# silencht/SG-SLAM

Hardware: AMD Instinct MI355X
Metric: tracked frames/sec (640x480 RGB-D) (higher is better)
Workload: dtype u8/f32(bf16x3 matrix products)/f64

## Files before the change

sg_slam_amd/csrc/sgx_flow.cpp:

```cpp
#include "sgx_flow_kernels.h"
#include "sgx_prof.h"
#include "sgx_stage.h"
#include "../../include/sgx.h"
#ifdef SGX_DEBUG_TAPS
#include "../../include/sgx_debug.h"
#endif
#include <stdio.h>
#include <stdlib.h>
#include <string.h>
#include <new>
#include <vector>

#define SGX_CHECK_HIP(expr) do { hipError_t _e = (expr); if (_e != hipSuccess) { \
    fprintf(stderr, "sgx: HIP error %d (%s) at %s:%d\n", (int)_e, hipGetErrorString(_e), __FILE__, __LINE__); return SGX_ERR_DEVICE; } } while (0)

struct sgx_flow {
    sgx_flow_config cfg;
    SgxLkGeom g;
    uint8_t *img[2] = { nullptr, nullptr };
    int cur = 0;
    int prev_batch = 0;
};

extern "C" int sgx_flow_create(const sgx_flow_config *cfg, sgx_flow **out)
{
    if (!cfg || !out) return SGX_ERR_INVALID;
    *out = nullptr;
    if (cfg->width < 1 || cfg->height < 1 || cfg->max_batch < 1 || cfg->max_count < 0 || !(cfg->epsilon >= 0)) return SGX_ERR_INVALID;
    if (cfg->win_size != SGX_LK_WIN || cfg->max_level < 0 || cfg->max_level >= SGX_LK_MAXL) return SGX_ERR_UNSUPPORTED;
    if (cfg->width <= 1 || cfg->height <= 1) return SGX_ERR_UNSUPPORTED;
    { const unsigned long long qw = (unsigned long long)((cfg->width + 3) >> 2); if (qw * qw * (unsigned long long)cfg->height >= (1ull << 32)) return SGX_ERR_UNSUPPORTED; }
    sgx_flow *h = new (std::nothrow) sgx_flow();
    if (!h) return SGX_ERR_NOMEM;
    h->cfg = *cfg;
    SgxLkGeom &g = h->g;
    memset(&g, 0, sizeof g);
    int w = cfg->width, hh = cfg->height; unsigned io = 0;
    for (int l = 0;; l++) {
        g.w[l] = w; g.h[l] = hh; g.pitch[l] = (w + 3) & ~3; g.ioff[l] = io;
        io += (unsigned)g.pitch[l] * (unsigned)hh;
        g.nl = l + 1;
        if (l == cfg->max_level) break;
        const int nw = (w + 1) / 2, nh = (hh + 1) / 2;
        if (nw <= cfg->win_size || nh <= cfg->win_size) break;
        w = nw; hh = nh;
    }
    g.img_stride = (io + 15u + 64u) & ~15u;
    for (int s = 0; s < 2; s++)
        if (hipMalloc((void **)&h->img[s], (size_t)g.img_stride * cfg->max_batch) != hipSuccess) { sgx_flow_destroy(h); return SGX_ERR_NOMEM; }
    *out = h;
    return SGX_OK;
}

extern "C" void sgx_flow_destroy(sgx_flow *h)
{
    if (!h) return;
    for (int s = 0; s < 2; s++) if (h->img[s]) (void)hipFree(h->img[s]);
    delete h;
}

extern "C" int sgx_flow_reset(sgx_flow *h) { if (!h) return SGX_ERR_INVALID; h->prev_batch = 0; return SGX_OK; }
extern "C" int sgx_flow_levels(const sgx_flow *h) { return h ? h->g.nl : SGX_ERR_INVALID; }

static int build_pyramid(sgx_flow *h, int slot, const uint8_t *d_gray, int pitch, int batch, sgx_stream_t st)
{
    const SgxLkGeom &g = h->g;
    uint8_t *base = h->img[slot];
    sgx_prof_begin(SGX_K_LK_PYR, st);
    auto magic = [](int d) -> unsigned { return d <= 1 ? 0u : (unsigned)((0x100000000ull + (unsigned)d - 1) / (unsigned)d); };
    SGX_LAUNCH(k_lk_copy, dim3(((g.pitch[0] >> 2) * g.h[0] + 255) / 256, batch), dim3(256), st, d_gray, g.w[0], g.h[0], pitch, base, g.pitch[0], g.img_stride, magic(g.pitch[0] >> 2));
    for (int l = 1; l < g.nl; l++)
        SGX_LAUNCH(k_lk_pyrdown, dim3(((g.pitch[l] >> 2) * g.h[l] + 255) / 256, batch), dim3(256), st, (const uint8_t *)(base + g.ioff[l - 1]), g.w[l - 1], g.h[l - 1], g.pitch[l - 1],
                   g.img_stride, base + g.ioff[l], g.w[l], g.h[l], g.pitch[l], g.img_stride, magic(g.pitch[l] >> 2));
    sgx_prof_end(SGX_K_LK_PYR, st);
    SGX_CHECK_HIP(hipGetLastError());
    return SGX_OK;
}

static int track(sgx_flow *h, int cur_slot, int prev_slot, int batch, const sgx_keypoint *d_keys, const int32_t *d_n, int cap, float *d_prev_xy, uint8_t *d_status, sgx_stream_t st)
{
    SgxLkArgs A;
    A.cur_img = h->img[cur_slot]; A.prev_img = h->img[prev_slot];
    A.keys = (const uint8_t *)d_keys; A.n = d_n; A.cap = cap; A.prev_xy = d_prev_xy; A.status = d_status;
    A.max_count = h->cfg.max_count > 100 ? 100 : h->cfg.max_count;
    double eps = h->cfg.epsilon > 10. ? 10. : h->cfg.epsilon;
    A.eps2 = eps * eps; A.min_eig = (float)1e-4;
    sgx_prof_begin(SGX_K_LK_TRACK, st);
    static const int kpw = sgx_getenv("SGX_LK_KPW") ? atoi(sgx_getenv("SGX_LK_KPW")) : 2;
    A.batch = batch; A.kblocks = (cap + 4 * kpw - 1) / (4 * kpw);
#ifdef SGX_DEBUG_TAPS
    if (kpw == 4) { auto kfn = k_lk_trackN<4>; SGX_LAUNCH(kfn, dim3((unsigned)A.kblocks * (unsigned)batch), dim3(256), st, h->g, A); }
    else if (kpw != 2) { A.kblocks = (cap + 3) / 4; SGX_LAUNCH(k_lk_track, dim3((unsigned)A.kblocks * (unsigned)batch), dim3(256), st, h->g, A); }
    else
#endif
    { auto kfn = k_lk_trackN<2>; SGX_LAUNCH(kfn, dim3((unsigned)A.kblocks * (unsigned)batch), dim3(256), st, h->g, A); }
    sgx_prof_end(SGX_K_LK_TRACK, st);
    SGX_CHECK_HIP(hipGetLastError());
    return SGX_OK;
}

extern "C" int sgx_flow_lk_batch_dev(sgx_flow *h, const uint8_t *d_gray, int pitch, int batch, const sgx_keypoint *d_keys, const int32_t *d_n, int cap,
                                     float *d_prev_xy, uint8_t *d_status, int32_t *have_prev, void *stream)
{
    if (!h || !d_gray || batch < 1 || batch > h->cfg.max_batch || pitch < h->cfg.width) return SGX_ERR_INVALID;
    if ((pitch & 3) || ((uintptr_t)d_gray & 3)) return SGX_ERR_INVALID;
    sgx_stream_t st = (sgx_stream_t)stream;
    const int cur = h->cur, prev = cur ^ 1;
    const bool tracked = h->prev_batch == batch;
    if (tracked && (!d_keys || !d_n || !d_prev_xy || cap < 1)) return SGX_ERR_INVALID;
    int rc = build_pyramid(h, cur, d_gray, pitch, batch, st);
    if (rc != SGX_OK) return rc;
    if (tracked) { rc = track(h, cur, prev, batch, d_keys, d_n, cap, d_prev_xy, d_status, st); if (rc != SGX_OK) return rc; }
    if (have_prev) *have_prev = tracked ? 1 : 0;
    h->cur = prev; h->prev_batch = batch;
    return SGX_OK;
}

extern "C" int sgx_flow_lk(sgx_flow *h, const uint8_t *gray_from, const uint8_t *gray_to, int stride, const float *pts, int n, float *next_pts, uint8_t *status)
{
    if (!h || !gray_from || !gray_to || stride < h->cfg.width || n < 0 || (n > 0 && (!pts || !next_pts))) return SGX_ERR_INVALID;
    if (n == 0) return SGX_OK;
    const int W = h->cfg.width, H = h->cfg.height, P = (W + 3) & ~3;
    std::vector<uint8_t> pack((size_t)P * H * 2, 0);
    for (int y = 0; y < H; y++) { memcpy(&pack[(size_t)y * P], gray_to + (size_t)y * stride, (size_t)W); memcpy(&pack[(size_t)(H + y) * P], gray_from + (size_t)y * stride, (size_t)W); }
    std::vector<sgx_keypoint> kp((size_t)n);
    for (int i = 0; i < n; i++) { memset(&kp[(size_t)i], 0, sizeof(sgx_keypoint)); kp[(size_t)i].x = pts[2 * i]; kp[(size_t)i].y = pts[2 * i + 1]; }
    SgxStaged dI, dK, dN, dO, dS;
    int rc;
    if ((rc = dI.put(0, pack.data(), pack.size())) != SGX_OK || (rc = dK.put(1, kp.data(), kp.size() * sizeof(sgx_keypoint))) != SGX_OK ||
        (rc = dN.put(2, &n, sizeof n)) != SGX_OK || (rc = dO.put(3, nullptr, (size_t)n * 8)) != SGX_OK || (rc = dS.put(4, nullptr, (size_t)n)) != SGX_OK) return rc;
    const int keep_cur = h->cur, keep_prev = h->prev_batch;
    if ((rc = build_pyramid(h, 1, (const uint8_t *)dI.p, P, 1, 0)) != SGX_OK) return rc;
    if ((rc = build_pyramid(h, 0, (const uint8_t *)dI.p + (size_t)P * H, P, 1, 0)) != SGX_OK) return rc;
    if ((rc = track(h, 0, 1, 1, (const sgx_keypoint *)dK.p, (const int32_t *)dN.p, n, (float *)dO.p, (uint8_t *)dS.p, 0)) != SGX_OK) return rc;
    SGX_CHECK_HIP(hipMemcpy(next_pts, dO.p, (size_t)n * 8, hipMemcpyDeviceToHost));
    if (status) SGX_CHECK_HIP(hipMemcpy(status, dS.p, (size_t)n, hipMemcpyDeviceToHost));
    h->cur = keep_cur; h->prev_batch = 0; (void)keep_prev;
    return SGX_OK;
}

SGX_TAP int sgx_flow_debug_read_level(sgx_flow *h, int slot, int frame, int level, uint8_t *img )
{
    if (!h || slot < 0 || slot > 1 || frame < 0 || frame >= h->cfg.max_batch || level < 0 || level >= h->g.nl) return SGX_ERR_INVALID;
    const SgxLkGeom &g = h->g;
    SGX_CHECK_HIP(hipDeviceSynchronize());
    if (!img) return SGX_ERR_INVALID;
    {
        std::vector<uint8_t> t((size_t)g.pitch[level] * g.h[level]);
        SGX_CHECK_HIP(hipMemcpy(t.data(), h->img[slot] + (size_t)frame * g.img_stride + g.ioff[level], t.size(), hipMemcpyDeviceToHost));
        for (int y = 0; y < g.h[level]; y++) memcpy(img + (size_t)y * g.w[level], &t[(size_t)y * g.pitch[level]], (size_t)g.w[level]);
    }
    return SGX_OK;
}
SGX_TAP int sgx_flow_debug_level_size(const sgx_flow *h, int level, int32_t *w, int32_t *hh)
{
    if (!h || level < 0 || level >= h->g.nl || !w || !hh) return SGX_ERR_INVALID;
    *w = h->g.w[level]; *hh = h->g.h[level];
    return SGX_OK;
}

#if defined(SGX_DEBUG_TAPS) && !defined(SGX_EMU)
typedef float sgx_dbg_f16v __attribute__((ext_vector_type(16)));
typedef __bf16 sgx_dbg_bf8 __attribute__((ext_vector_type(8)));
SGX_KERNEL_OCC(256, 2) k_dbg_corun_bf16(float *o, int iters)
{
    const uint32_t x = threadIdx.x * 2654435761u + blockIdx.x, y = x ^ 0x9e3779b9u;
    sgx_dbg_f16v acc = {0}; sgx_dbg_bf8 a, b;
    for (int i = 0; i < 8; i++) { a[i] = (__bf16)(float)((x >> i) & 7); b[i] = (__bf16)(float)((y >> i) & 3); }
    for (int i = 0; i < iters; i++) acc = __builtin_amdgcn_mfma_f32_32x32x16_bf16(a, b, acc, 0, 0, 0);
    float s = 0.f; for (int i = 0; i < 16; i++) s += acc[i];
    o[(blockIdx.x & 1023) * 256 + threadIdx.x] = s;
}
#endif
SGX_TAP int sgx_debug_corun_bf16(int blocks, int iters, int launches, void *stream)
{
#if defined(SGX_DEBUG_TAPS) && !defined(SGX_EMU)
    static float *sink = nullptr;
    if (blocks < 1 || iters < 1 || launches < 1) return SGX_ERR_INVALID;
    if (!sink) SGX_CHECK_HIP(hipMalloc((void **)&sink, 1024 * 256 * sizeof(float)));
    for (int l = 0; l < launches; l++) SGX_LAUNCH(k_dbg_corun_bf16, dim3((unsigned)blocks), dim3(256), (sgx_stream_t)stream, sink, iters);
    SGX_CHECK_HIP(hipGetLastError());
    return SGX_OK;
#else
    (void)blocks; (void)iters; (void)launches; (void)stream;
    return SGX_ERR_UNSUPPORTED;
#endif
}

extern "C" int sgx_fundamental_ransac_batch_dev(int batch, int cap, const sgx_keypoint *d_keys, const int32_t *d_n, const float *d_prev_xy,
                                                const int32_t *d_pre_have_dynamic, const float *d_pre_boxes, const int32_t *d_pre_nboxes, int max_boxes,
                                                double threshold, double confidence, double *d_F, int32_t *d_ok, int32_t *d_stats, void *stream)
{
    if (batch < 1 || cap < 1 || !d_keys || !d_n || !d_prev_xy || !d_F || !d_ok || max_boxes < 0) return SGX_ERR_INVALID;
    if (cap > SGX_FM_MAXPTS) return SGX_ERR_UNSUPPORTED;
    SgxFmArgs A;
    A.keys = (const uint8_t *)d_keys; A.n = d_n; A.cap = cap; A.prev_xy = d_prev_xy;
    A.pre_have = d_pre_have_dynamic; A.pre_boxes = d_pre_boxes; A.pre_nboxes = d_pre_nboxes; A.max_boxes = max_boxes;
    if (threshold <= 0) threshold = 3;
    if (confidence < DBL_EPSILON || confidence > 1 - DBL_EPSILON) confidence = 0.99;
    A.threshold = threshold; A.confidence = confidence; A.max_iters = 1000;
    A.F = d_F; A.ok = d_ok; A.stats = d_stats;
    const size_t lds = (size_t)cap * 16 + 1024 + (((size_t)cap + 15) & ~(size_t)15);
    sgx_prof_begin(SGX_K_FM_RANSAC, (sgx_stream_t)stream);
    SGX_LAUNCH_DYN(k_fm_ransac, dim3(batch), dim3(256), lds, (sgx_stream_t)stream, A);
    sgx_prof_end(SGX_K_FM_RANSAC, (sgx_stream_t)stream);
    SGX_CHECK_HIP(hipGetLastError());
    return SGX_OK;
}

extern "C" int sgx_find_fundamental_mat(const float *pts1, const float *pts2, int n, double threshold, double confidence, double *F, int32_t *ok, int32_t *stats)
{
    if (n < 0 || (n > 0 && (!pts1 || !pts2)) || !F || !ok) return SGX_ERR_INVALID;
    if (n > SGX_FM_MAXPTS) return SGX_ERR_UNSUPPORTED;
    const int cap = n > 0 ? n : 1;
    std::vector<sgx_keypoint> kp((size_t)cap);
    memset(kp.data(), 0, kp.size() * sizeof(sgx_keypoint));
    for (int i = 0; i < n; i++) { kp[(size_t)i].x = pts1[2 * i]; kp[(size_t)i].y = pts1[2 * i + 1]; }
    SgxStaged dK, dN, dP, dF, dO, dS;
    int rc;
    if ((rc = dK.put(0, kp.data(), kp.size() * sizeof(sgx_keypoint))) != SGX_OK || (rc = dN.put(1, &n, sizeof n)) != SGX_OK ||
        (rc = dP.put(2, n ? pts2 : nullptr, (size_t)cap * 8)) != SGX_OK || (rc = dF.put(3, nullptr, 72)) != SGX_OK || (rc = dO.put(4, nullptr, 4)) != SGX_OK ||
        (rc = dS.put(5, nullptr, 16)) != SGX_OK) return rc;
    rc = sgx_fundamental_ransac_batch_dev(1, cap, (const sgx_keypoint *)dK.p, (const int32_t *)dN.p, (const float *)dP.p, nullptr, nullptr, nullptr, 0, threshold, confidence,
                                          (double *)dF.p, (int32_t *)dO.p, (int32_t *)dS.p, nullptr);
    if (rc != SGX_OK) return rc;
    SGX_CHECK_HIP(hipMemcpy(F, dF.p, 72, hipMemcpyDeviceToHost));
    SGX_CHECK_HIP(hipMemcpy(ok, dO.p, 4, hipMemcpyDeviceToHost));
    if (stats) SGX_CHECK_HIP(hipMemcpy(stats, dS.p, 16, hipMemcpyDeviceToHost));
    return SGX_OK;
}
```

sg_slam_amd/csrc/sgx_flow_kernels.h:

```cpp
#pragma once
#include "sgx_rt.h"
#include "sgx_block.h"
#include <float.h>
#include <math.h>

#define SGX_LK_MAXL 4
#define SGX_LK_WIN 21
#define SGX_LK_TILE_PITCH 36
struct SgxLkGeom {
    int nl;
    int w[SGX_LK_MAXL], h[SGX_LK_MAXL], pitch[SGX_LK_MAXL];
    unsigned ioff[SGX_LK_MAXL];
    unsigned img_stride;
};

SGX_DEV int sgx_reflect101(int p, int len)
{
    if (len == 1) return 0;
    while (p < 0 || p >= len) { if (p < 0) p = -p; else p = 2 * len - 2 - p; }
    return p;
}
SGX_DEV int sgx_floor_f(float v) { return (int)floorf(v); }
SGX_DEV float sgx_i64_to_f32(long long v)
{
    const long long hi = v >> 24; const int lo = (int)(v - (hi << 24));
    return (float)(int)hi * 16777216.0f + (float)lo;
}

SGX_DEV unsigned sgx_lk_udiv(unsigned n, unsigned m)
{
#ifndef SGX_EMU
    return m ? __umulhi(n, m) : n;
#else
    return m ? (unsigned)(((unsigned long long)n * m) >> 32) : n;
#endif
}
SGX_KERNEL(256) k_lk_copy(const uint8_t *src, int w, int h, int spitch, uint8_t *dst, int dpitch, unsigned dstride, unsigned qw_magic)
{
    SGX_THREADS_BEGIN(tid)
    const int f = (int)blockIdx.y, qw = dpitch >> 2, q = (int)blockIdx.x * 256 + tid;
    if (q < qw * h) {
        const int y = (int)sgx_lk_udiv((unsigned)q, qw_magic), x = (q - y * qw) * 4;
        const uint8_t *s = src + ((size_t)f * h + y) * spitch;
        uint32_t v;
        if (x + 4 <= w) v = *(const uint32_t *)(s + x);
        else { v = 0; for (int i = 0; x + i < w; i++) v |= (uint32_t)s[x + i] << (8 * i); }
        *(uint32_t *)(dst + (size_t)f * dstride + (size_t)y * dpitch + x) = v;
    }
    SGX_THREADS_END
}

SGX_KERNEL(256) k_lk_pyrdown(const uint8_t *src, int sw, int sh, int spitch, unsigned sstride, uint8_t *dst, int dw, int dh, int dpitch, unsigned dstride, unsigned qw_magic)
{
    SGX_THREADS_BEGIN(tid)
    const int f = (int)blockIdx.y, qw = dpitch >> 2, q = (int)blockIdx.x * 256 + tid;
    if (q < qw * dh) {
        const int y = (int)sgx_lk_udiv((unsigned)q, qw_magic), X = (q - y * qw) * 4;
        const uint8_t *S = src + (size_t)f * sstride;
        int acc[4] = { 0, 0, 0, 0 };
        const bool fast = X >= 2 && 2 * X + 11 < spitch && 2 * X + 8 <= sw - 1;
#pragma unroll
        for (int k = 0; k < 5; k++) {
            const int wk = k == 0 || k == 4 ? 1 : k == 2 ? 6 : 4;
            const uint8_t *row = S + (size_t)sgx_reflect101(2 * y - 2 + k, sh) * spitch;
            int p[11];
            if (fast) {
                const uint32_t *r4 = (const uint32_t *)(row + 2 * X - 4);
                const uint32_t a = r4[0], b = r4[1], c = r4[2], d = r4[3];
                p[0] = (a >> 16) & 255; p[1] = a >> 24;
                p[2] = b & 255; p[3] = (b >> 8) & 255; p[4] = (b >> 16) & 255; p[5] = b >> 24;
                p[6] = c & 255; p[7] = (c >> 8) & 255; p[8] = (c >> 16) & 255; p[9] = c >> 24;
                p[10] = d & 255;
            } else {
#pragma unroll
                for (int i = 0; i < 11; i++) p[i] = row[sgx_reflect101(2 * X - 2 + i, sw)];
            }
#pragma unroll
            for (int o = 0; o < 4; o++) acc[o] += wk * (p[2 * o + 2] * 6 + (p[2 * o + 1] + p[2 * o + 3]) * 4 + p[2 * o] + p[2 * o + 4]);
        }
        uint32_t out = 0;
#pragma unroll
        for (int o = 0; o < 4; o++) out |= (uint32_t)((acc[o] + 128) >> 8) << (8 * o);
        *(uint32_t *)(dst + (size_t)f * dstride + (size_t)y * dpitch + X) = out;
    }
    SGX_THREADS_END
}

struct SgxLkWeights { int w00, w01, w10, w11; };
SGX_DEV SgxLkWeights sgx_lk_weights(float a, float b)
{
    SgxLkWeights k;
    k.w00 = sgx_cvround((1.f - a) * (1.f - b) * (float)(1 << 14));
    k.w01 = sgx_cvround(a * (1.f - b) * (float)(1 << 14));
    k.w10 = sgx_cvround((1.f - a) * b * (float)(1 << 14));
    k.w11 = (1 << 14) - k.w00 - k.w01 - k.w10;
    return k;
}
#define SGX_LK_DESCALE(x, n) (((x) + (1 << ((n) - 1))) >> (n))

struct SgxLkStep { float dx, dy; };
SGX_DEV SgxLkStep sgx_lk_step(float A11, float A12, float A22, float D, long long sb1, long long sb2)
{
    const float FLT_SCALE = 1.f / (1 << 20);
    const float b1 = sgx_i64_to_f32(sb1) * FLT_SCALE, b2 = sgx_i64_to_f32(sb2) * FLT_SCALE;
    SgxLkStep s;
    s.dx = (A12 * b2 - A22 * b1) * D;
    s.dy = (A12 * b1 - A11 * b2) * D;
    return s;
}

struct SgxLkArgs {
    const uint8_t *cur_img, *prev_img;
    const uint8_t *keys; const int *n; int cap;
    float *prev_xy; uint8_t *status;
    int max_count; double eps2; float min_eig;
    int batch, kblocks;
};
SGX_DEV void sgx_lk_decode_block(int i, int batch, int kblocks, int &f, int &kb)
{
    const int full = (batch / 8) * 8;
    if (i < full * kblocks) { const int x = i & 7, j = i >> 3; kb = j % kblocks; f = x + 8 * (j / kblocks); }
    else { const int j = i - full * kblocks; f = full + j / kblocks; kb = j % kblocks; }
}

#ifdef SGX_EMU
static inline int sgx_lk_px(const uint8_t *I, int w, int h, int pitch, int x, int y) { return I[(size_t)sgx_reflect101(y, h) * pitch + sgx_reflect101(x, w)]; }
static void sgx_lk_track_point(const SgxLkGeom &g, const uint8_t *I0, const uint8_t *J0, float kx, float ky, int max_count, double eps2, float min_eig,
                               float *ox, float *oy, uint8_t *ost)
{
    const int W = SGX_LK_WIN; const float half = (W - 1) * 0.5f, FLT_SCALE = 1.f / (1 << 20);
    float outx = 0.f, outy = 0.f; uint8_t status = 1;
    static thread_local short Iw[SGX_LK_WIN * SGX_LK_WIN], dIw[SGX_LK_WIN * SGX_LK_WIN * 2];
    for (int level = g.nl - 1; level >= 0; level--) {
        const int w = g.w[level], h = g.h[level], pitch = g.pitch[level];
        const uint8_t *I = I0 + g.ioff[level], *J = J0 + g.ioff[level];
        const float sc = 1.0f / (float)(1 << level);
        float prevx = kx * sc, prevy = ky * sc, nextx, nexty;
        if (level == g.nl - 1) { nextx = prevx; nexty = prevy; } else { nextx = outx * 2.f; nexty = outy * 2.f; }
        outx = nextx; outy = nexty;
        prevx -= half; prevy -= half;
        const int ipx = sgx_floor_f(prevx), ipy = sgx_floor_f(prevy);
        if (ipx < -W || ipx >= w || ipy < -W || ipy >= h) { if (level == 0) status = 0; continue; }
        SgxLkWeights k = sgx_lk_weights(prevx - ipx, prevy - ipy);
        long long s11 = 0, s12 = 0, s22 = 0;
        for (int y = 0; y < W; y++) for (int x = 0; x < W; x++) {
            int pv[4], dx[4], dy[4];
            for (int c = 0; c < 4; c++) {
                const int gx = ipx + x + (c & 1), gy = ipy + y + (c >> 1);
                pv[c] = sgx_lk_px(I, w, h, pitch, gx, gy);
                if (gx < 0 || gy < 0 || gx >= w || gy >= h) { dx[c] = dy[c] = 0; }
                else {
                    int t0[3], t1[3];
                    for (int q = 0; q < 3; q++) {
                        const int a = sgx_lk_px(I, w, h, pitch, gx - 1 + q, gy - 1), b = sgx_lk_px(I, w, h, pitch, gx - 1 + q, gy), cc = sgx_lk_px(I, w, h, pitch, gx - 1 + q, gy + 1);
                        t0[q] = (a + cc) * 3 + b * 10; t1[q] = cc - a;
                    }
                    dx[c] = t0[2] - t0[0]; dy[c] = (t1[0] + t1[2]) * 3 + t1[1] * 10;
                }
            }
            const int iv = SGX_LK_DESCALE(pv[0] * k.w00 + pv[1] * k.w01 + pv[2] * k.w10 + pv[3] * k.w11, 9);
            const int ix = SGX_LK_DESCALE(dx[0] * k.w00 + dx[1] * k.w01 + dx[2] * k.w10 + dx[3] * k.w11, 14);
            const int iy = SGX_LK_DESCALE(dy[0] * k.w00 + dy[1] * k.w01 + dy[2] * k.w10 + dy[3] * k.w11, 14);
            Iw[y * W + x] = (short)iv; dIw[(y * W + x) * 2] = (short)ix; dIw[(y * W + x) * 2 + 1] = (short)iy;
            s11 += (long long)ix * ix; s12 += (long long)ix * iy; s22 += (long long)iy * iy;
        }
        const float A11 = sgx_i64_to_f32(s11) * FLT_SCALE, A12 = sgx_i64_to_f32(s12) * FLT_SCALE, A22 = sgx_i64_to_f32(s22) * FLT_SCALE;
        float D = A11 * A22 - A12 * A12;
        const float minEig = (A22 + A11 - sqrtf((A11 - A22) * (A11 - A22) + 4.f * A12 * A12)) / (float)(2 * W * W);
        if (minEig < min_eig || D < FLT_EPSILON) { if (level == 0) status = 0; continue; }
        D = 1.f / D;
        nextx -= half; nexty -= half;
        float pdx = 0.f, pdy = 0.f;
        for (int j = 0; j < max_count; j++) {
            const int inx = sgx_floor_f(nextx), iny = sgx_floor_f(nexty);
            if (inx < -W || inx >= w || iny < -W || iny >= h) { if (level == 0) status = 0; break; }
            k = sgx_lk_weights(nextx - inx, nexty - iny);
            long long sb1 = 0, sb2 = 0;
            for (int y = 0; y < W; y++) for (int x = 0; x < W; x++) {
                int pv[4];
                for (int c = 0; c < 4; c++) pv[c] = sgx_lk_px(J, w, h, pitch, inx + x + (c & 1), iny + y + (c >> 1));
                const int diff = SGX_LK_DESCALE(pv[0] * k.w00 + pv[1] * k.w01 + pv[2] * k.w10 + pv[3] * k.w11, 9) - Iw[y * W + x];
                sb1 += (long long)diff * dIw[(y * W + x) * 2]; sb2 += (long long)diff * dIw[(y * W + x) * 2 + 1];
            }
            const SgxLkStep st = sgx_lk_step(A11, A12, A22, D, sb1, sb2);
            nextx += st.dx; nexty += st.dy;
            outx = nextx + half; outy = nexty + half;
            if ((double)st.dx * st.dx + (double)st.dy * st.dy <= eps2) break;
            if (j > 0 && fabs((double)(st.dx + pdx)) < 0.01 && fabs((double)(st.dy + pdy)) < 0.01) { outx -= st.dx * 0.5f; outy -= st.dy * 0.5f; break; }
            pdx = st.dx; pdy = st.dy;
        }
        if (status && level == 0) {
            const int ix = sgx_floor_f(outx - half), iy = sgx_floor_f(outy - half);
            if (ix < -W || ix >= w || iy < -W || iy >= h) status = 0;
        }
    }
    *ox = outx; *oy = outy; *ost = status;
}
SGX_KERNEL(256) k_lk_track(SgxLkGeom g, SgxLkArgs A)
{
    SGX_THREADS_BEGIN(tid)
    int f, kb;
    sgx_lk_decode_block((int)blockIdx.x, A.batch, A.kblocks, f, kb);
    const int kp = kb * 4 + (tid >> 6);
    if ((tid & 63) == 0 && kp < A.n[f] && kp < A.cap) {
        const float *kpt = (const float *)(A.keys + ((size_t)f * A.cap + kp) * 28);
        float ox, oy; uint8_t st;
        sgx_lk_track_point(g, A.cur_img + (size_t)f * g.img_stride, A.prev_img + (size_t)f * g.img_stride, kpt[0], kpt[1], A.max_count, A.eps2, A.min_eig, &ox, &oy, &st);
        A.prev_xy[2 * ((size_t)f * A.cap + kp)] = ox; A.prev_xy[2 * ((size_t)f * A.cap + kp) + 1] = oy;
        if (A.status) A.status[(size_t)f * A.cap + kp] = st;
    }
    SGX_THREADS_END
}
#else
SGX_DEV int sgx_wave_sum_i32(int v)
{
    v += __builtin_amdgcn_update_dpp(0, v, 0xB1, 0xF, 0xF, true);
    v += __builtin_amdgcn_update_dpp(0, v, 0x4E, 0xF, 0xF, true);
    v += __builtin_amdgcn_update_dpp(0, v, 0x124, 0xF, 0xF, true);
    v += __builtin_amdgcn_update_dpp(0, v, 0x128, 0xF, 0xF, true);
    v += __builtin_amdgcn_update_dpp(0, v, 0x142, 0xA, 0xF, false);
    v += __builtin_amdgcn_update_dpp(0, v, 0x143, 0xC, 0xF, false);
    return __builtin_amdgcn_readlane(v, 63);
}
SGX_DEV float sgx_wave_sum_f32(int v)
{
    const int lo = sgx_wave_sum_i32(v & 0xFFFF), hi = sgx_wave_sum_i32(v >> 16);
    return fmaf((float)hi, 65536.0f, (float)lo);
}
SGX_DEV int sgx_mul24(int a, int b) { return __mul24(a, b); }
SGX_DEV int sgx_reflect1(int p, int len) { p = p < 0 ? -p : p; p = p >= len ? 2 * len - 2 - p : p; return min(max(p, 0), len - 1); }

typedef short sgx_i16x2 __attribute__((ext_vector_type(2)));
typedef unsigned short sgx_u16x2 __attribute__((ext_vector_type(2)));
SGX_DEV sgx_i16x2 sgx_as_i16x2(uint32_t v) { return __builtin_bit_cast(sgx_i16x2, v); }
SGX_DEV uint32_t sgx_as_u32(sgx_i16x2 v) { return __builtin_bit_cast(uint32_t, v); }
#define SGX_LK_PAIR(hi, lo, a, b) sgx_as_i16x2(__builtin_amdgcn_perm((hi), (lo), (uint32_t)(a) | 0x0c00u | ((uint32_t)(b) << 16) | 0x0c000000u))
SGX_DEV sgx_i16x2 sgx_lk_next(sgx_i16x2 p, sgx_i16x2 q) { return sgx_as_i16x2(__builtin_amdgcn_alignbit(sgx_as_u32(q), sgx_as_u32(p), 16)); }
#if defined(SGX_LK_NODOT) && !defined(SGX_EMU)
SGX_DEV int sgx_lk_dot2_mad(sgx_i16x2 a, sgx_i16x2 b, int c)
{
    const uint32_t ua = __builtin_bit_cast(uint32_t, a), ub = __builtin_bit_cast(uint32_t, b);
    asm("v_mad_i32_i16 %0, %1, %2, %0 op_sel:[0,0,0,0]" : "+v"(c) : "v"(ua), "v"(ub));
    asm("v_mad_i32_i16 %0, %1, %2, %0 op_sel:[1,1,0,0]" : "+v"(c) : "v"(ua), "v"(ub));
    return c;
}
#define SGX_LK_DOT2(a, b, c) sgx_lk_dot2_mad((a), (b), (c))
#else
#define SGX_LK_DOT2(a, b, c) __builtin_amdgcn_sdot2((a), (b), (c), false)
#endif
SGX_DEV int sgx_lk_dot2_keep(sgx_i16x2 a, sgx_i16x2 b, int c) { return SGX_LK_DOT2(a, b, c); }

template <int PASSES>
SGX_DEV void sgx_lk_stage(uint32_t *tile, const uint8_t *img, int w, int h, int pitch, int ox, int oy, int rl, int cl)
{
    __builtin_amdgcn_fence(__ATOMIC_SEQ_CST, "wavefront"); __builtin_amdgcn_wave_barrier();
    const int gx = ox + 4 * cl;
    const bool inside = gx >= 0 && gx + 4 <= w;
    if (rl < 7) {
        uint32_t v[PASSES];
        if (inside) {
#pragma unroll
            for (int p = 0; p < PASSES; p++) v[p] = *(const uint32_t *)(img + (size_t)sgx_reflect1(oy + p * 7 + rl, h) * pitch + gx);
        } else {
            const int x0 = sgx_reflect1(gx, w), x1 = sgx_reflect1(gx + 1, w), x2 = sgx_reflect1(gx + 2, w), x3 = sgx_reflect1(gx + 3, w);
#pragma unroll
            for (int p = 0; p < PASSES; p++) {
                const uint8_t *src = img + (size_t)sgx_reflect1(oy + p * 7 + rl, h) * pitch;
                v[p] = (uint32_t)src[x0] | ((uint32_t)src[x1] << 8) | ((uint32_t)src[x2] << 16) | ((uint32_t)src[x3] << 24);
            }
        }
#pragma unroll
        for (int p = 0; p < PASSES; p++) tile[(p * 7 + rl) * (SGX_LK_TILE_PITCH / 4) + cl] = v[p];
    }
    __builtin_amdgcn_fence(__ATOMIC_SEQ_CST, "wavefront"); __builtin_amdgcn_wave_barrier();
}

#ifdef SGX_DEBUG_TAPS
SGX_KERNEL(256) k_lk_track(SgxLkGeom g, SgxLkArgs A)
{
    __shared__ uint32_t tiles[4][35 * SGX_LK_TILE_PITCH / 4 + 5];
    const int tid = (int)threadIdx.x, lane = tid & 63, wv = tid >> 6;
    int f, kb;
    sgx_lk_decode_block((int)blockIdx.x, A.batch, A.kblocks, f, kb);
    const int kp = kb * 4 + wv;
    if (kp >= A.n[f] || kp >= A.cap) return;
    uint32_t *tile = tiles[wv];
    const uint8_t *tile8 = (const uint8_t *)tile;
    const int W = SGX_LK_WIN; const float half = 10.0f, FLT_SCALE = 1.f / (1 << 20);
    const float *kpt = (const float *)(A.keys + ((size_t)f * A.cap + kp) * 28);
    const float kx = __builtin_bit_cast(float, __builtin_amdgcn_readfirstlane(__builtin_bit_cast(int, kpt[0])));
    const float ky = __builtin_bit_cast(float, __builtin_amdgcn_readfirstlane(__builtin_bit_cast(int, kpt[1])));
    const uint8_t *I0 = A.cur_img + (size_t)f * g.img_stride, *J0 = A.prev_img + (size_t)f * g.img_stride;
    const int r = lane / 3, s7 = (lane - 3 * r) * 7;
    const int rl = lane / 9, cl = lane - 9 * rl;
    const bool active = lane < 63;
    const int lane_off = active ? r * SGX_LK_TILE_PITCH + s7 : 0;
    float outx = 0.f, outy = 0.f; int status = 1;

    for (int level = g.nl - 1; level >= 0; level--) {
        const int w = g.w[level], h = g.h[level], pitch = g.pitch[level];
        const uint8_t *I = I0 + g.ioff[level], *J = J0 + g.ioff[level];
        const float sc = 1.0f / (float)(1 << level);
        float prevx = kx * sc, prevy = ky * sc, nextx, nexty;
        if (level == g.nl - 1) { nextx = prevx; nexty = prevy; } else { nextx = outx * 2.f; nexty = outy * 2.f; }
        outx = nextx; outy = nexty;
        prevx -= half; prevy -= half;
        const int ipx = sgx_floor_f(prevx), ipy = sgx_floor_f(prevy);
        if (ipx < -W || ipx >= w || ipy < -W || ipy >= h) { if (level == 0) status = 0; continue; }
        SgxLkWeights k = sgx_lk_weights(prevx - ipx, prevy - ipy);
        sgx_i16x2 W0 = sgx_as_i16x2((uint32_t)k.w00 | ((uint32_t)k.w01 << 16)), W1 = sgx_as_i16x2((uint32_t)k.w10 | ((uint32_t)k.w11 << 16));

        int ivb[7]; int ix[7], iy[7];
        int s11 = 0, s12 = 0, s22 = 0;
        {
            const int gy0 = ipy + r, gx0 = ipx + s7;
            sgx_i16x2 P[4][5];
            const bool direct = ipx >= 1 && ipx + 25 < w && ipy >= 1 && ipy + 22 < h;
            if (direct) {
                const uint8_t *gb = I + (size_t)(active ? gy0 - 1 : ipy) * pitch + (active ? gx0 - 1 : ipx);
#pragma unroll
                for (int j = 0; j < 4; j++) {
                    uint32_t q[3];
                    __builtin_memcpy(q, gb + (size_t)j * pitch, 12);
                    P[j][0] = SGX_LK_PAIR(q[0], q[0], 0, 1); P[j][1] = SGX_LK_PAIR(q[0], q[0], 2, 3);
                    P[j][2] = SGX_LK_PAIR(q[1], q[1], 0, 1); P[j][3] = SGX_LK_PAIR(q[1], q[1], 2, 3);
                    P[j][4] = SGX_LK_PAIR(q[2], q[2], 0, 1);
                }
            } else {
                const int tx = ((ipx - 1) >> 2) << 2, ty = ipy - 1;
                sgx_lk_stage<4>(tile, I, w, h, pitch, tx, ty, rl, cl);
                const uint8_t *tb = tile8 + lane_off + (ipx - 1 - tx);
#pragma unroll
                for (int j = 0; j < 4; j++) {
                    uint32_t q[3];
                    __builtin_memcpy(q, tb + j * SGX_LK_TILE_PITCH, 12);
                    P[j][0] = SGX_LK_PAIR(q[0], q[0], 0, 1); P[j][1] = SGX_LK_PAIR(q[0], q[0], 2, 3);
                    P[j][2] = SGX_LK_PAIR(q[1], q[1], 0, 1); P[j][3] = SGX_LK_PAIR(q[1], q[1], 2, 3);
                    P[j][4] = SGX_LK_PAIR(q[2], q[2], 0, 1);
                }
            }
            const sgx_i16x2 c3 = { 3, 3 }, c10 = { 10, 10 };
            const sgx_i16x2 Wd0 = active ? W0 : sgx_as_i16x2(0u), Wd1 = active ? W1 : sgx_as_i16x2(0u);
            sgx_i16x2 S0[5], S1[5], D0[5], D1[5];
#pragma unroll
            for (int q = 0; q < 5; q++) {
                S0[q] = (P[0][q] + P[2][q]) * c3 + P[1][q] * c10; D0[q] = P[2][q] - P[0][q];
                S1[q] = (P[1][q] + P[3][q]) * c3 + P[2][q] * c10; D1[q] = P[3][q] - P[1][q];
            }
            sgx_i16x2 xa[5], ya[5], xb[5], yb[5];
            const bool whole = ipx >= 0 && ipx + W < w && ipy >= 0 && ipy + W < h;
#pragma unroll
            for (int q = 0; q < 4; q++) {
                xa[q] = S0[q + 1] - S0[q]; ya[q] = (D0[q] + D0[q + 1]) * c3 + sgx_lk_next(D0[q], D0[q + 1]) * c10;
                xb[q] = S1[q + 1] - S1[q]; yb[q] = (D1[q] + D1[q + 1]) * c3 + sgx_lk_next(D1[q], D1[q + 1]) * c10;
            }
            if (!whole) {
                const bool rowa = gy0 >= 0 && gy0 < h, rowb = gy0 + 1 >= 0 && gy0 + 1 < h;
#pragma unroll
                for (int q = 0; q < 4; q++) {
                    const int x = gx0 + 2 * q;
                    const uint32_t m = ((x >= 0 && x < w) ? 0xFFFFu : 0u) | ((x + 1 >= 0 && x + 1 < w) ? 0xFFFF0000u : 0u);
                    const uint32_t ma = rowa ? m : 0u, mb = rowb ? m : 0u;
                    xa[q] = sgx_as_i16x2(sgx_as_u32(xa[q]) & ma); ya[q] = sgx_as_i16x2(sgx_as_u32(ya[q]) & ma);
                    xb[q] = sgx_as_i16x2(sgx_as_u32(xb[q]) & mb); yb[q] = sgx_as_i16x2(sgx_as_u32(yb[q]) & mb);
                }
            }
#pragma unroll
            for (int c = 0; c < 7; c++) {
                const sgx_i16x2 pxa = (c & 1) ? sgx_lk_next(xa[c >> 1], xa[(c >> 1) + 1]) : xa[c >> 1], pxb = (c & 1) ? sgx_lk_next(xb[c >> 1], xb[(c >> 1) + 1]) : xb[c >> 1];
                const sgx_i16x2 pya = (c & 1) ? sgx_lk_next(ya[c >> 1], ya[(c >> 1) + 1]) : ya[c >> 1], pyb = (c & 1) ? sgx_lk_next(yb[c >> 1], yb[(c >> 1) + 1]) : yb[c >> 1];
                const sgx_i16x2 pia = (c & 1) ? P[1][(c + 1) >> 1] : sgx_lk_next(P[1][c >> 1], P[1][(c >> 1) + 1]), pib = (c & 1) ? P[2][(c + 1) >> 1] : sgx_lk_next(P[2][c >> 1], P[2][(c >> 1) + 1]);
                const int v = SGX_LK_DOT2(pib, W1, SGX_LK_DOT2(pia, W0, 256)) >> 9;
                const int vx = SGX_LK_DOT2(pxb, Wd1, SGX_LK_DOT2(pxa, Wd0, 8192)) >> 14;
                const int vy = SGX_LK_DOT2(pyb, Wd1, SGX_LK_DOT2(pya, Wd0, 8192)) >> 14;
                ivb[c] = 256 - (v << 9); ix[c] = vx; iy[c] = vy;
                s11 += sgx_mul24(vx, vx); s12 += sgx_mul24(vx, vy); s22 += sgx_mul24(vy, vy);
            }
        }
        const float A11 = sgx_wave_sum_f32(s11) * FLT_SCALE, A12 = sgx_wave_sum_f32(s12) * FLT_SCALE, A22 = sgx_wave_sum_f32(s22) * FLT_SCALE;
        float D = A11 * A22 - A12 * A12;
        const float minEig = (A22 + A11 - sqrtf((A11 - A22) * (A11 - A22) + 4.f * A12 * A12)) / (float)(2 * W * W);
        if (minEig < A.min_eig || D < FLT_EPSILON) { if (level == 0) status = 0; continue; }
        D = 1.f / D;
        nextx -= half; nexty -= half;
        float pdx = 0.f, pdy = 0.f;
        int ox = 0, oy = 0; bool staged = false;
// ... 667 lines not shown
```

Before: 28440.

## Fuse LK pyramid levels: tiled copy+pyrdown and LDS-resident levels 2-3

Replaces the separate level-0 copy and level-1 pyrdown with a tiled kernel that loads a source tile into LDS, writes the level-0 copy from it and computes level 1 from the same tile. Levels 2 and 3 are built by a single 1024-thread block per frame that stages level 1 in dynamic LDS and keeps level 2 in LDS for level 3. This removes kernel launches and global round-trips between levels. The cost is one block per frame for the small levels, which gives low parallelism, plus a large dynamic LDS allocation that only fits when the levels are small enough.

New measurement: 28660, median of 6. Within noise of the previous version (+0.8%).

```diff
diff --git a/sg_slam_amd/csrc/sgx_flow.cpp b/sg_slam_amd/csrc/sgx_flow.cpp
--- a/sg_slam_amd/csrc/sgx_flow.cpp
+++ b/sg_slam_amd/csrc/sgx_flow.cpp
@@ -20,6 +20,7 @@
     uint8_t *img[2] = { nullptr, nullptr };
     int cur = 0;
     int prev_batch = 0;
+    size_t pyr_lds = 0;
 };
 
 extern "C" int sgx_flow_create(const sgx_flow_config *cfg, sgx_flow **out)
@@ -46,6 +47,15 @@
         w = nw; hh = nh;
     }
     g.img_stride = (io + 15u + 64u) & ~15u;
+    if (g.nl >= 3) {
+        const size_t need = (size_t)g.pitch[1] * g.h[1] + (g.nl > 3 ? (size_t)g.pitch[2] * g.h[2] : 0);
+        if (need <= 144 * 1024) {
+            h->pyr_lds = need;
+#ifndef SGX_EMU
+            if (hipFuncSetAttribute((const void *)k_lk_pyr23, hipFuncAttributeMaxDynamicSharedMemorySize, (int)need) != hipSuccess) { delete h; return SGX_ERR_DEVICE; }
+#endif
+        }
+    }
     for (int s = 0; s < 2; s++)
         if (hipMalloc((void **)&h->img[s], (size_t)g.img_stride * cfg->max_batch) != hipSuccess) { sgx_flow_destroy(h); return SGX_ERR_NOMEM; }
     *out = h;
@@ -68,10 +78,18 @@
     uint8_t *base = h->img[slot];
     sgx_prof_begin(SGX_K_LK_PYR, st);
     auto magic = [](int d) -> unsigned { return d <= 1 ? 0u : (unsigned)((0x100000000ull + (unsigned)d - 1) / (unsigned)d); };
-    SGX_LAUNCH(k_lk_copy, dim3(((g.pitch[0] >> 2) * g.h[0] + 255) / 256, batch), dim3(256), st, d_gray, g.w[0], g.h[0], pitch, base, g.pitch[0], g.img_stride, magic(g.pitch[0] >> 2));
-    for (int l = 1; l < g.nl; l++)
+    auto pyrdown = [&](int l) {
         SGX_LAUNCH(k_lk_pyrdown, dim3(((g.pitch[l] >> 2) * g.h[l] + 255) / 256, batch), dim3(256), st, (const uint8_t *)(base + g.ioff[l - 1]), g.w[l - 1], g.h[l - 1], g.pitch[l - 1],
                    g.img_stride, base + g.ioff[l], g.w[l], g.h[l], g.pitch[l], g.img_stride, magic(g.pitch[l] >> 2));
+    };
+    if (g.nl < 2 || batch > 65535)
+        SGX_LAUNCH(k_lk_copy, dim3(((g.pitch[0] >> 2) * g.h[0] + 255) / 256, batch), dim3(256), st, d_gray, g.w[0], g.h[0], pitch, base, g.pitch[0], g.img_stride, magic(g.pitch[0] >> 2));
+    else
+        SGX_LAUNCH(k_lk_pyr01, dim3((g.pitch[1] + SGX_PYR_TW - 1) / SGX_PYR_TW, (g.h[1] + SGX_PYR_TH - 1) / SGX_PYR_TH, batch), dim3(256), st, d_gray, pitch, g.w[0], g.h[0], g.pitch[0],
+                   g.h[1], g.pitch[1], g.ioff[1], g.img_stride, base);
+    if (g.nl >= 2 && batch > 65535) pyrdown(1);
+    if (g.nl >= 3 && h->pyr_lds) SGX_LAUNCH_DYN(k_lk_pyr23, dim3(batch), dim3(1024), h->pyr_lds, st, g, base);
+    else for (int l = 2; l < g.nl; l++) pyrdown(l);
     sgx_prof_end(SGX_K_LK_PYR, st);
     SGX_CHECK_HIP(hipGetLastError());
     return SGX_OK;
diff --git a/sg_slam_amd/csrc/sgx_flow_kernels.h b/sg_slam_amd/csrc/sgx_flow_kernels.h
--- a/sg_slam_amd/csrc/sgx_flow_kernels.h
+++ b/sg_slam_amd/csrc/sgx_flow_kernels.h
@@ -50,38 +50,124 @@
     SGX_THREADS_END
 }
 
+SGX_DEV void sgx_lk_pyr_row(int (&acc)[4], const int (&p)[11], int k)
+{
+    const int wk = k == 0 || k == 4 ? 1 : k == 2 ? 6 : 4;
+#pragma unroll
+    for (int o = 0; o < 4; o++) acc[o] += wk * (p[2 * o + 2] * 6 + (p[2 * o + 1] + p[2 * o + 3]) * 4 + p[2 * o] + p[2 * o + 4]);
+}
+SGX_DEV void sgx_lk_pyr_unpack(int (&p)[11], uint32_t a, uint32_t b, uint32_t c, uint32_t d)
+{
+    p[0] = (a >> 16) & 255; p[1] = a >> 24;
+    p[2] = b & 255; p[3] = (b >> 8) & 255; p[4] = (b >> 16) & 255; p[5] = b >> 24;
+    p[6] = c & 255; p[7] = (c >> 8) & 255; p[8] = (c >> 16) & 255; p[9] = c >> 24;
+    p[10] = d & 255;
+}
+SGX_DEV uint32_t sgx_lk_pyr_pack(const int (&acc)[4])
+{
+    uint32_t out = 0;
+#pragma unroll
+    for (int o = 0; o < 4; o++) out |= (uint32_t)((acc[o] + 128) >> 8) << (8 * o);
+    return out;
+}
+SGX_DEV uint32_t sgx_lk_pyrdown_quad(const uint8_t *S, int sw, int sh, int spitch, int X, int y)
+{
+    int acc[4] = { 0, 0, 0, 0 };
+    const bool fast = X >= 2 && 2 * X + 11 < spitch && 2 * X + 8 <= sw - 1;
+#pragma unroll
+    for (int k = 0; k < 5; k++) {
+        const uint8_t *row = S + (size_t)sgx_reflect101(2 * y - 2 + k, sh) * spitch;
+        int p[11];
+        if (fast) {
+            const uint32_t *r4 = (const uint32_t *)(row + 2 * X - 4);
+            sgx_lk_pyr_unpack(p, r4[0], r4[1], r4[2], r4[3]);
+        } else {
+#pragma unroll
+            for (int i = 0; i < 11; i++) p[i] = row[sgx_reflect101(2 * X - 2 + i, sw)];
+        }
+        sgx_lk_pyr_row(acc, p, k);
+    }
+    return sgx_lk_pyr_pack(acc);
+}
 SGX_KERNEL(256) k_lk_pyrdown(const uint8_t *src, int sw, int sh, int spitch, unsigned sstride, uint8_t *dst, int dw, int dh, int dpitch, unsigned dstride, unsigned qw_magic)
 {
     SGX_THREADS_BEGIN(tid)
     const int f = (int)blockIdx.y, qw = dpitch >> 2, q = (int)blockIdx.x * 256 + tid;
     if (q < qw * dh) {
         const int y = (int)sgx_lk_udiv((unsigned)q, qw_magic), X = (q - y * qw) * 4;
-        const uint8_t *S = src + (size_t)f * sstride;
+        *(uint32_t *)(dst + (size_t)f * dstride + (size_t)y * dpitch + X) = sgx_lk_pyrdown_quad(src + (size_t)f * sstride, sw, sh, spitch, X, y);
+    }
+    SGX_THREADS_END
+}
+
+#define SGX_PYR_TW 64
+#define SGX_PYR_TH 16
+#define SGX_PYR_SP (2 * SGX_PYR_TW / 4 + 2)
+#define SGX_PYR_SR (2 * SGX_PYR_TH + 3)
+SGX_KERNEL(256) k_lk_pyr01(const uint8_t *src, int spitch, int w, int h, int pitch0, int h1, int pitch1, unsigned ioff1, unsigned dstride, uint8_t *dst)
+{
+    SGX_LDS uint32_t tile[SGX_PYR_SR * SGX_PYR_SP];
+    const int f = (int)blockIdx.z, X0 = (int)blockIdx.x * SGX_PYR_TW, y0 = (int)blockIdx.y * SGX_PYR_TH;
+    const uint8_t *S = src + (size_t)f * h * spitch;
+    uint8_t *D = dst + (size_t)f * dstride;
+    SGX_THREADS_BEGIN(tid)
+    for (int i = tid; i < SGX_PYR_SR * SGX_PYR_SP; i += 256) {
+        const int r = i / SGX_PYR_SP, cq = i - r * SGX_PYR_SP;
+        const int gy = 2 * y0 - 2 + r, gx = 2 * X0 - 4 + 4 * cq;
+        const uint8_t *row = S + (size_t)sgx_reflect101(gy, h) * spitch;
+        uint32_t v;
+        if (gx >= 0 && gx + 4 <= w) v = *(const uint32_t *)(row + gx);
+        else { v = 0; for (int b = 0; b < 4; b++) v |= (uint32_t)row[sgx_reflect101(gx + b, w)] << (8 * b); }
+        tile[i] = v;
+        if (r >= 2 && r < SGX_PYR_SR - 1 && gy < h && cq >= 1 && cq < SGX_PYR_SP - 1 && gx < pitch0) {
+            if (gx + 4 > w) v &= (1u << (8 * (w - gx))) - 1u;
+            *(uint32_t *)(D + (size_t)gy * pitch0 + gx) = v;
+        }
+    }
+    SGX_THREADS_END
+    SGX_SYNC();
+    SGX_THREADS_BEGIN(tid)
+    const int q = tid & 15, ry = tid >> 4, y = y0 + ry, X = X0 + 4 * q;
+    if (y < h1 && X < pitch1) {
         int acc[4] = { 0, 0, 0, 0 };
-        const bool fast = X >= 2 && 2 * X + 11 < spitch && 2 * X + 8 <= sw - 1;
 #pragma unroll
         for (int k = 0; k < 5; k++) {
-            const int wk = k == 0 || k == 4 ? 1 : k == 2 ? 6 : 4;
-            const uint8_t *row = S + (size_t)sgx_reflect101(2 * y - 2 + k, sh) * spitch;
+            const uint32_t *t = tile + (2 * ry + k) * SGX_PYR_SP + 2 * q;
             int p[11];
-            if (fast) {
-                const uint32_t *r4 = (const uint32_t *)(row + 2 * X - 4);
-                const uint32_t a = r4[0], b = r4[1], c = r4[2], d = r4[3];
-                p[0] = (a >> 16) & 255; p[1] = a >> 24;
-                p[2] = b & 255; p[3] = (b >> 8) & 255; p[4] = (b >> 16) & 255; p[5] = b >> 24;
-                p[6] = c & 255; p[7] = (c >> 8) & 255; p[8] = (c >> 16) & 255; p[9] = c >> 24;
-                p[10] = d & 255;
-            } else {
-#pragma unroll
-                for (int i = 0; i < 11; i++) p[i] = row[sgx_reflect101(2 * X - 2 + i, sw)];
-            }
-#pragma unroll
-            for (int o = 0; o < 4; o++) acc[o] += wk * (p[2 * o + 2] * 6 + (p[2 * o + 1] + p[2 * o + 3]) * 4 + p[2 * o] + p[2 * o + 4]);
-        }
-        uint32_t out = 0;
-#pragma unroll
-        for (int o = 0; o < 4; o++) out |= (uint32_t)((acc[o] + 128) >> 8) << (8 * o);
-        *(uint32_t *)(dst + (size_t)f * dstride + (size_t)y * dpitch + X) = out;
+            sgx_lk_pyr_unpack(p, t[0], t[1], t[2], t[3]);
+            sgx_lk_pyr_row(acc, p, k);
+        }
+        *(uint32_t *)(D + ioff1 + (size_t)y * pitch1 + X) = sgx_lk_pyr_pack(acc);
+    }
+    SGX_THREADS_END
+}
+
+SGX_KERNEL(1024) k_lk_pyr23(SgxLkGeom g, uint8_t *dst)
+{
+    SGX_DYN_LDS(lds);
+    uint8_t *D = dst + (size_t)blockIdx.x * g.img_stride;
+    uint8_t *L1 = lds, *L2 = lds + (size_t)g.pitch[1] * g.h[1];
+    SGX_THREADS_BEGIN(tid)
+    const int n1 = (g.pitch[1] >> 2) * g.h[1];
+    for (int i = tid; i < n1; i += 1024) ((uint32_t *)L1)[i] = ((const uint32_t *)(D + g.ioff[1]))[i];
+    SGX_THREADS_END
+    SGX_SYNC();
+    SGX_THREADS_BEGIN(tid)
+    const int qw = g.pitch[2] >> 2, n2 = qw * g.h[2];
+    for (int i = tid; i < n2; i += 1024) {
+        const int y = i / qw, X = (i - y * qw) * 4;
+        const uint32_t v = sgx_lk_pyrdown_quad(L1, g.w[1], g.h[1], g.pitch[1], X, y);
+        ((uint32_t *)(D + g.ioff[2]))[i] = v;
+        if (g.nl > 3) ((uint32_t *)L2)[i] = v;
+    }
+    SGX_THREADS_END
+    if (g.nl <= 3) return;
+    SGX_SYNC();
+    SGX_THREADS_BEGIN(tid)
+    const int qw = g.pitch[3] >> 2, n3 = qw * g.h[3];
+    for (int i = tid; i < n3; i += 1024) {
+        const int y = i / qw, X = (i - y * qw) * 4;
+        ((uint32_t *)(D + g.ioff[3]))[i] = sgx_lk_pyrdown_quad(L2, g.w[2], g.h[2], g.pitch[2], X, y);
     }
     SGX_THREADS_END
 }
```
